# TaceoLabs/collaborative-circom

Hardware: AMD Instinct MI355X
Metric: Groth16 constraints/sec (BN254, 2^22 R1CS), one REP3 party's prove (higher is better)
Workload: dtype u32; 1 GPU; synthetic R1CS 2^22 constraints-domain BN254, REP3 co-groth16 (configs[2]); num_constraints=4194302, domain_size=4194304, nnz=12582906, msm=8 G1 + 2 G2 of ~2^22 points, ntt=12

## Files before the change

collaborative-circom_amd/csrc/capi_internal.hpp:

```cpp
#pragma once
#include "common.hpp"
#include "launchers.hpp"
#include "curve.hpp"
#include "subgroup.hpp"
#include "host_ec64.hpp"
#include "ntt_kernels.hpp"
#include "plonk_kernels.hpp"

#include <cmath>
#include <chrono>
#include <map>
#include <set>
#include <mutex>
#include <vector>

using namespace cg;

hipError_t hip_malloc_flush(void** p, size_t bytes);
template <class T> hipError_t hip_malloc_flush(T** p, size_t bytes) { return hip_malloc_flush((void**)p, bytes); }

namespace cgi {

struct Arena {
    char* base = nullptr; size_t cap = 0, used = 0;
    void* take(size_t bytes) { void* p = base + used; used += align_up(bytes); return p; }
};

enum { TW_BITREV = 1, TW_NATURAL = 2 };
struct TwKey { int curve; int log_m; uint32_t gen[8]; int kind = 0;
    bool operator<(const TwKey& o) const { if (curve != o.curve) return curve < o.curve; if (log_m != o.log_m) return log_m < o.log_m; if (kind != o.kind) return kind < o.kind; return memcmp(gen, o.gen, sizeof gen) < 0; } };
struct CosetKey { TwKey k; uint32_t scale[8]; bool operator<(const CosetKey& o) const { if (k < o.k) return true; if (o.k < k) return false; return memcmp(scale, o.scale, sizeof scale) < 0; } };
struct CosetTables { void* lo; void* hi; int log_lo; };

enum { TAG_MSM = 0, TAG_NTT, TAG_VEC, TAG_SPMV, TAG_SORT, TAG_ACC_G1, TAG_ACC_G2, TAG_REDUCE, TAG_COUNT };
struct EvPair { hipEvent_t a, b; int tag; };

struct MsmTicket {
    bool live = false;
    int curve = 0, group = 0, k = 0, c = 0, nwin = 0;
    uint32_t* h_flags = nullptr; bool optimistic = false;
    const cg_bases* bases = nullptr; size_t offset = 0, n = 0; std::vector<const void*> scalars;
    int nsums = 0;
    bool plain_fold = false;
    bool bit_fold = false;
    bool grid_fold = false; int log_l = 0, log_h = 0; uint32_t gc = 1, gr = 1;
    void* h_pinned = nullptr; size_t pinned_bytes = 0;
    hipEvent_t done = nullptr;
};

}
using namespace cgi;


struct cg_ctx {
    int device = 0;
    hipStream_t stream = nullptr;
    bool owns_stream = true;
    hipStream_t aux = nullptr;
    static constexpr int ACC_SLOTS_MAX = 8;
    hipEvent_t ev_acc[ACC_SLOTS_MAX] = {}, ev_red[ACC_SLOTS_MAX] = {};
    bool slot_busy[ACC_SLOTS_MAX] = {};
// ... 158 lines not shown
```

collaborative-circom_amd/csrc/capi_ntt.hip:

```cpp
#include "capi_internal.hpp"

namespace {
template <class Fr>
void host_pow_tables(const Fr& w, const Fr& first, int log_lo, size_t hi_n, std::vector<Fr>& lo, std::vector<Fr>& hi) {
    lo.resize((size_t)1 << log_lo); hi.resize(hi_n);
    Fr acc = first, step = Fr::one();
    for (size_t j = 0; j < lo.size(); j++) { lo[j] = acc; acc = acc * w; step = step * w; }
    Fr h = Fr::one();
    for (size_t j = 0; j < hi_n; j++) { hi[j] = h; h = h * step; }
}

struct SharedTwiddles { void* p; size_t bytes; int refs; uint64_t stamp; };
std::mutex g_tw_mu;
std::map<std::pair<int, TwKey>, SharedTwiddles> g_tw;
uint64_t g_tw_clock = 0;
void* shared_twiddles_acquire(int device, const TwKey& key) {
    std::lock_guard<std::mutex> l(g_tw_mu);
    auto it = g_tw.find({device, key});
    if (it == g_tw.end()) return nullptr;
    it->second.refs++; it->second.stamp = ++g_tw_clock;
    return it->second.p;
}
void* shared_twiddles_publish(int device, const TwKey& key, void* p, size_t bytes) {
    std::lock_guard<std::mutex> l(g_tw_mu);
// ... 49 lines not shown
    HIPCHK(hipStreamSynchronize(ctx->stream));
    HIPCHK(hipFree(d_lo)); HIPCHK(hipFree(d_hi));
    d_tw = shared_twiddles_publish(ctx->device, key, d_tw, bytes);
    ctx->twiddles[key] = d_tw;
    *out = d_tw;
    return 0;
}

template <class Fr>
int get_coset_tables(cg_ctx* ctx, int curve, int log_m, const Fr& g, const Fr& scale, CosetTables* out) {
    CosetKey key; key.k.curve = curve; key.k.log_m = log_m; memcpy(key.k.gen, g.v, sizeof key.k.gen); memcpy(key.scale, scale.v, sizeof key.scale);
    auto it = ctx->cosets.find(key);
    if (it != ctx->cosets.end()) { *out = it->second; return 0; }
    const size_t m = (size_t)1 << log_m;
    const int log_lo = std::min(11, log_m);
    const size_t hi_n = std::max<size_t>(1, m >> log_lo);
    std::vector<Fr> lo, hi;
    host_pow_tables(g, scale, log_lo, hi_n, lo, hi);
    CosetTables t; t.log_lo = log_lo;
    HIPCHK(hip_malloc_flush(&t.lo, lo.size() * sizeof(Fr)));
    HIPCHK(hip_malloc_flush(&t.hi, hi.size() * sizeof(Fr)));
    HIPCHK(hipMemcpy(t.lo, lo.data(), lo.size() * sizeof(Fr), hipMemcpyHostToDevice));
    HIPCHK(hipMemcpy(t.hi, hi.data(), hi.size() * sizeof(Fr), hipMemcpyHostToDevice));
    if (ctx->cosets.size() >= 64) {
        HIPCHK(hipStreamSynchronize(ctx->stream));
        for (auto& kv : ctx->cosets) { hipFree(kv.second.lo); hipFree(kv.second.hi); }
        ctx->cosets.clear();
    }
    ctx->cosets[key] = t;
    *out = t;
    return 0;
}

struct NttPass { int s0, k, t; };
std::vector<NttPass> ntt_plan(int log_m, int tile_log) {
    std::vector<NttPass> plan;
    const int k_last = std::min(log_m, tile_log);
    const int rest = log_m - k_last;
    int s0 = 0;
    if (rest > 0) {
        const int np = (rest + 6) / 7;
        for (int i = 0; i < np; i++) {
            int k = rest / np + (i < rest % np ? 1 : 0);
            plan.push_back({s0, k, tile_log - k});
            s0 += k;
        }
    }
    plan.push_back({s0, k_last, 0});
    return plan;
}

int ntt_lazy_tile() {
    static const int tile = [] { const char* e = tune_env("CG_NTT_TILE"); const int v = e ? atoi(e) : NTT_TILE_LOG_LAZY; return std::min(NTT_TILE_LOG, std::max(8, v)); }();
    return tile;
}

template <class Fr>
int ntt_run(cg_ctx* ctx, int curve, void* const* d_vecs, int k, size_t n, const Fr& gen, bool inverse, const Fr* coset, size_t arena_off) {
    const int log_m = log2_floor(n);
    if (((size_t)1 << log_m) != n) return fail(CG_ERR_ARG, "NTT length must be a power of two");
    if (k < 1 || k > NTT_MAX_VECS) return fail(CG_ERR_ARG, "k out of range");
    if (n == 1) return 0;
    if (!inverse && coset) return fail(CG_ERR_ARG, "coset_gen is only supported with inverse != 0");
    const Fr w = inverse ? fp_inverse(gen) : gen;
    const void* twl = nullptr;
    int rc = get_twiddles_lazy<Fr>(ctx, curve, log_m, w, false, &twl);
    if (rc) return rc;
    NttVecs data{}, tmp{};
    for (int j = 0; j < k; j++) { data.p[j] = d_vecs[j]; tmp.p[j] = ctx->ntt_arena.base + arena_off + (size_t)j * lazy29_bytes(n); }
    hipStream_t st = ctx->stream;
    bool first = true;
    for (const NttPass& p : ntt_plan(log_m, ntt_lazy_tile())) { rc = launch_ntt_ct_pass<Fr>(st, first, first ? data : tmp, tmp, k, n, log_m, p.s0, p.k, p.t, twl); if (rc) return rc; first = false; }
    const Fr scale32 = inverse ? mont32<Fr>() * inv_pow2<Fr>(log_m) : mont32<Fr>();
    CosetTables t;
    const Fr* d_scale = nullptr; const Fr* c_lo = nullptr; const Fr* c_hi = nullptr; int log_lo = 0;
    if (coset) { rc = get_coset_tables<Fr>(ctx, curve, log_m, *coset, scale32, &t); if (rc) return rc; c_lo = (const Fr*)t.lo; c_hi = (const Fr*)t.hi; log_lo = t.log_lo; }
    else { rc = get_coset_tables<Fr>(ctx, curve, 0, Fr::one(), scale32, &t); if (rc) return rc; d_scale = (const Fr*)t.lo; }
    return launch_bitrev_finish_lazy<Fr>(st, data, tmp, k, n, log_m, d_scale, c_lo, c_hi, log_lo);
}

template <class Fr>
int ntt_coset_pair_run(cg_ctx* ctx, int curve, void* const* d_vecs, int k, size_t n, const Fr& gen, const Fr& coset, size_t arena_off) {
    const int log_m = log2_floor(n);
    if (((size_t)1 << log_m) != n) return fail(CG_ERR_ARG, "NTT length must be a power of two");
    if (k < 1 || k > NTT_MAX_VECS) return fail(CG_ERR_ARG, "k out of range");
    if (n == 1) return 0;
    const void* tw_inv = nullptr; const void* tw_fwd = nullptr;
    int rc = get_twiddles_lazy<Fr>(ctx, curve, log_m, fp_inverse(gen), false, &tw_inv); if (rc) return rc;
    rc = get_twiddles_lazy<Fr>(ctx, curve, log_m, gen, true, &tw_fwd); if (rc) return rc;
    const Fr c32 = mont32<Fr>();
    CosetTables ct;
    rc = get_coset_tables<Fr>(ctx, curve, log_m, coset, c32 * inv_pow2<Fr>(log_m), &ct); if (rc) return rc;
    NttVecs data{}, tmp{};
    for (int j = 0; j < k; j++) { data.p[j] = d_vecs[j]; tmp.p[j] = ctx->ntt_arena.base + arena_off + (size_t)j * lazy29_bytes(n); }
    hipStream_t st = ctx->stream;
    const std::vector<NttPass> plan = ntt_plan(log_m, ntt_lazy_tile());
    bool first = true;
    for (const NttPass& p : plan) { rc = launch_ntt_ct_pass<Fr>(st, first, first ? data : tmp, tmp, k, n, log_m, p.s0, p.k, p.t, tw_inv); if (rc) return rc; first = false; }
    for (size_t i = plan.size(); i-- > 0;) {
        const NttPass& p = plan[i];
        rc = launch_ntt_dit_pass<Fr>(st, i + 1 == plan.size(), i == 0, data, tmp, k, n, log_m, p.s0, p.k, p.t, tw_fwd, (const Fr*)ct.lo, (const Fr*)ct.hi, ct.log_lo, c32);
        if (rc) return rc;
    }
    return 0;
}

}

extern "C" {
int32_t cg_ntt_dev(cg_ctx* ctx, int32_t curve, void* const* d_vecs, int32_t k, size_t n, const void* h_group_gen, int32_t inverse, const void* h_coset_gen) {
    if (!ctx || !d_vecs || !h_group_gen) return fail(CG_ERR_ARG, "null argument");
    HIPCHK(hipSetDevice(ctx->device));
    return with_fr(curve, [&](auto tag) -> int {
        typedef decltype(tag) Fr;
        Fr gen, cos; copy_in(gen, h_group_gen);
        if (h_coset_gen) copy_in(cos, h_coset_gen);
        if (n > 1) { int rc = ensure_ntt_arena(ctx, (size_t)k * lazy29_bytes(n)); if (rc) return rc; }
        StatScope ss(ctx, TAG_NTT);
        return ntt_run<Fr>(ctx, curve, d_vecs, k, n, gen, inverse != 0, h_coset_gen ? &cos : nullptr, 0);
    });
}
int32_t cg_ntt_coset_pair_dev(cg_ctx* ctx, int32_t curve, void* const* d_vecs, int32_t k, size_t n, const void* h_group_gen, const void* h_coset_gen) {
    if (!ctx || !d_vecs || !h_group_gen || !h_coset_gen) return fail(CG_ERR_ARG, "null argument");
    HIPCHK(hipSetDevice(ctx->device));
    return with_fr(curve, [&](auto tag) -> int {
        typedef decltype(tag) Fr;
        Fr gen, cos; copy_in(gen, h_group_gen); copy_in(cos, h_coset_gen);
        if (n > 1) { int rc = ensure_ntt_arena(ctx, (size_t)k * lazy29_bytes(n)); if (rc) return rc; }
        StatScope ss(ctx, TAG_NTT);
        return ntt_coset_pair_run<Fr>(ctx, curve, d_vecs, k, n, gen, cos, 0);
    });
}
int32_t cg_ntt(cg_ctx* ctx, int32_t curve, void* const* h_vecs, int32_t k, size_t n, const void* h_group_gen, int32_t inverse, const void* h_coset_gen) {
    if (!ctx || !h_vecs) return fail(CG_ERR_ARG, "null argument");
// ... 28 lines not shown
```

collaborative-circom_amd/csrc/fr_impl.hpp:

```cpp
#pragma once
#include "launchers.hpp"
#include "ntt_kernels.hpp"
#include "vec_kernels.hpp"
#include "plonk_kernels.hpp"
#include "r1cs_kernels.hpp"
#include "plonk_setup_kernels.hpp"
#include "msm_sort_kernels.hpp"

namespace cg {

template <class Fr> int launch_vec_binary(hipStream_t st, int op, Fr* out, const Fr* a, const Fr* b, size_t n) {
    if (!n) return 0;
    if (op == 0) hipLaunchKernelGGL((k_vec_binary<Fr, 0>), dim3(grid_for(n)), dim3(256), 0, st, out, a, b, n);
    else if (op == 1) hipLaunchKernelGGL((k_vec_binary<Fr, 1>), dim3(grid_for(n)), dim3(256), 0, st, out, a, b, n);
    else hipLaunchKernelGGL((k_vec_binary<Fr, 2>), dim3(grid_for(n)), dim3(256), 0, st, out, a, b, n);
    HIPCHK(hipGetLastError());
    return 0;
}
template <class Fr> int launch_rep3_mul_local(hipStream_t st, Fr* out, const Fr* aa, const Fr* ab, const Fr* ba, const Fr* bb, const Fr* mask, size_t n) {
    if (!n) return 0;
    hipLaunchKernelGGL((k_rep3_mul_local<Fr>), dim3(grid_for(n)), dim3(256), 0, st, out, aa, ab, ba, bb, mask, n);
    HIPCHK(hipGetLastError());
    return 0;
}
// ... 129 lines not shown
    for (int i = 0; i < 5; i++) if (n > n_constraints) HIPCHK(hipMemsetAsync((Fr*)o.q[i] + n_constraints, 0, (n - n_constraints) * sizeof(Fr), st));
    if (n_rows + n_public) hipLaunchKernelGGL((k_plonk_gate_emit<Fr>), dim3(grid_for(n_rows + n_public)), dim3(256), 0, st, A, B, C, n_rows, n_wires, n_public, counts, offsets, o);
    HIPCHK(hipGetLastError());
    return 0;
}
template <class Fr> int launch_plonk_sigma_labels(hipStream_t st, const uint32_t* prev, const Fr* wpow, int log_n, const Fr& k1, const Fr& k2, Fr* sigma) {
    hipLaunchKernelGGL((k_plonk_sigma_labels<Fr>), dim3(grid_for((size_t)3 << log_n)), dim3(256), 0, st, prev, wpow, log_n, k1, k2, sigma);
    HIPCHK(hipGetLastError());
    return 0;
}
template <class Fr> int launch_build_twiddles_lazy(hipStream_t st, void* tw, size_t m, int log_m, const Fr* lo, const Fr* hi, int log_lo, const Fr& c32) {
    if (m > 1) hipLaunchKernelGGL((k_build_twiddles_lazy<Fr>), dim3(grid_for(m / 2)), dim3(256), 0, st, tw, m / 2, log_m, lo, hi, log_lo, c32);
    HIPCHK(hipGetLastError());
    return 0;
}
template <class Fr> int launch_ntt_ct_pass(hipStream_t st, bool first, NttVecs src, NttVecs dst, int nvec, size_t n, int log_m, int s0, int k, int t, const void* tw) {
    static PerDeviceOnce attr_set;
    if (attr_set.pending()) {
        HIPCHK(hipFuncSetAttribute((const void*)k_ntt_ct_pass<Fr, true>, hipFuncAttributeMaxDynamicSharedMemorySize, 36 << NTT_TILE_LOG));
        HIPCHK(hipFuncSetAttribute((const void*)k_ntt_ct_pass<Fr, false>, hipFuncAttributeMaxDynamicSharedMemorySize, 36 << NTT_TILE_LOG));
        attr_set.mark();
    }
    const int E = 1 << (k + t);
    if (first) hipLaunchKernelGGL((k_ntt_ct_pass<Fr, true>), dim3((unsigned)(n / E), nvec), dim3(NTT_THREADS), (size_t)E * 36, st, src, dst, log_m, s0, k, t, tw);
    else hipLaunchKernelGGL((k_ntt_ct_pass<Fr, false>), dim3((unsigned)(n / E), nvec), dim3(NTT_THREADS), (size_t)E * 36, st, src, dst, log_m, s0, k, t, tw);
    HIPCHK(hipGetLastError());
    return 0;
}
template <class Fr> int launch_build_twiddles_lazy_natural(hipStream_t st, void* tw, size_t m, const Fr* lo, const Fr* hi, int log_lo, const Fr& c32) {
    if (m > 1) hipLaunchKernelGGL((k_build_twiddles_lazy_natural<Fr>), dim3(grid_for(m / 2)), dim3(256), 0, st, tw, m / 2, lo, hi, log_lo, c32);
    HIPCHK(hipGetLastError());
    return 0;
}
template <class Fr> int launch_ntt_dit_pass(hipStream_t st, bool first, bool last, NttVecs out, NttVecs tmp, int nvec, size_t n, int log_m, int s0, int k, int t, const void* tw,
                                            const Fr* c_lo, const Fr* c_hi, int log_lo, const Fr& c32) {
    static PerDeviceOnce attr_set;
    if (attr_set.pending()) {
        HIPCHK(hipFuncSetAttribute((const void*)k_ntt_dit_pass<Fr, true, true>, hipFuncAttributeMaxDynamicSharedMemorySize, 36 << NTT_TILE_LOG));
        HIPCHK(hipFuncSetAttribute((const void*)k_ntt_dit_pass<Fr, true, false>, hipFuncAttributeMaxDynamicSharedMemorySize, 36 << NTT_TILE_LOG));
        HIPCHK(hipFuncSetAttribute((const void*)k_ntt_dit_pass<Fr, false, true>, hipFuncAttributeMaxDynamicSharedMemorySize, 36 << NTT_TILE_LOG));
        HIPCHK(hipFuncSetAttribute((const void*)k_ntt_dit_pass<Fr, false, false>, hipFuncAttributeMaxDynamicSharedMemorySize, 36 << NTT_TILE_LOG));
        attr_set.mark();
    }
    const int E = 1 << (k + t);
    const dim3 grid((unsigned)(n / E), nvec); const size_t lds = (size_t)E * 36;
    if (first && last) hipLaunchKernelGGL((k_ntt_dit_pass<Fr, true, true>), grid, dim3(NTT_THREADS), lds, st, out, tmp, log_m, s0, k, t, tw, c_lo, c_hi, log_lo, c32);
    else if (first) hipLaunchKernelGGL((k_ntt_dit_pass<Fr, true, false>), grid, dim3(NTT_THREADS), lds, st, out, tmp, log_m, s0, k, t, tw, c_lo, c_hi, log_lo, c32);
    else if (last) hipLaunchKernelGGL((k_ntt_dit_pass<Fr, false, true>), grid, dim3(NTT_THREADS), lds, st, out, tmp, log_m, s0, k, t, tw, c_lo, c_hi, log_lo, c32);
    else hipLaunchKernelGGL((k_ntt_dit_pass<Fr, false, false>), grid, dim3(NTT_THREADS), lds, st, out, tmp, log_m, s0, k, t, tw, c_lo, c_hi, log_lo, c32);
    HIPCHK(hipGetLastError());
    return 0;
}
template <class Fr> int launch_bitrev_finish_lazy(hipStream_t st, NttVecs dst, NttVecs src, int nvec, size_t n, int log_m, const Fr* scale, const Fr* c_lo, const Fr* c_hi, int log_lo) {
    if (log_m >= 2 * BITREV_B_LAZY)
        hipLaunchKernelGGL((k_bitrev_finish_lazy<Fr>), dim3((unsigned)(n >> (2 * BITREV_B_LAZY)), nvec), dim3(256), 0, st, dst, src, log_m, scale, c_lo, c_hi, log_lo);
    else
        hipLaunchKernelGGL((k_bitrev_finish_lazy_small<Fr>), dim3(grid_for(n), nvec), dim3(256), 0, st, dst, src, log_m, scale, c_lo, c_hi, log_lo);
    HIPCHK(hipGetLastError());
    return 0;
}

inline bool msm_sort_use_partition(size_t n, int c, int nwin, int shared) {
    const size_t nbuckets = (size_t)(shared ? 1 : nwin) << (c - 1);
    const size_t nregions = (nbuckets + ((size_t)1 << PART_REGION_LOG) - 1) >> PART_REGION_LOG;
    return (size_t)nwin * n >= ((size_t)1 << 21) && nregions >= 8 && nregions <= PART_MAX_REGIONS;
}
template <class Fr> int msm_sort_launch(hipStream_t st, const Fr* d_scalars, size_t n, int c, int nwin, int shared, char* scratch, MsmSortPtrs* out, hipEvent_t* evs) {
    const size_t nbuckets = (size_t)(shared ? 1 : nwin) << (c - 1);
    size_t off = 0;
    auto take = [&](size_t bytes) { void* p = scratch + off; off += align_up(bytes); return p; };
    int32_t* digits = (int32_t*)take((size_t)nwin * n * 4);
    uint32_t* sorted = (uint32_t*)take((size_t)nwin * n * 4);
    uint32_t* counts = (uint32_t*)take(nbuckets * 4);
    uint32_t* cursors = (uint32_t*)take(nbuckets * 4);
    uint32_t* offsets = (uint32_t*)take(nbuckets * 4);
    const size_t ntiles = (nbuckets + SCAN_TILE - 1) / SCAN_TILE;
    uint32_t* tile_sums = (uint32_t*)take(ntiles * 4);
    if (evs) HIPCHK(hipEventRecord(evs[0], st));
    const bool no_small = !global_option(CG_GOPT_SORT_SMALL);
    static PerDeviceOnce attr_small; static std::atomic<bool> small_unavailable{false};
    if (shared && !no_small && !small_unavailable.load(std::memory_order_relaxed) && attr_small.pending()) {
        if (hipFuncSetAttribute((const void*)k_msm_sort_small<Fr>, hipFuncAttributeMaxDynamicSharedMemorySize, (int)((2 * SORT_SMALL_MAX_BUCKETS + 1024) * 4)) == hipSuccess) attr_small.mark();
// ... 78 lines not shown
}

#define CG_INSTANTIATE_FR(Fr)                                                                                              \
    namespace cg {                                                                                                         \
    template decltype(launch_vec_binary<Fr>) launch_vec_binary<Fr>;                                                        \
    template decltype(launch_rep3_mul_local<Fr>) launch_rep3_mul_local<Fr>;                                                \
    template decltype(launch_distribute_powers<Fr>) launch_distribute_powers<Fr>;                                          \
    template decltype(launch_vec_count_noncanonical<Fr>) launch_vec_count_noncanonical<Fr>;                                \
    template decltype(launch_vec_fill<Fr>) launch_vec_fill<Fr>;                                                            \
    template decltype(launch_vec_gather_idx<Fr>) launch_vec_gather_idx<Fr>;                                                \
    template decltype(launch_vec_affine<Fr>) launch_vec_affine<Fr>;                                                        \
    template decltype(launch_vec_gather_strided<Fr>) launch_vec_gather_strided<Fr>;                                        \
    template decltype(launch_vec_lincomb<Fr>) launch_vec_lincomb<Fr>;                                                      \
    template decltype(launch_shamir_share<Fr>) launch_shamir_share<Fr>;                                                    \
    template decltype(launch_plonk_r2_factors<Fr>) launch_plonk_r2_factors<Fr>;                                            \
    template decltype(launch_prefix_scan<Fr>) launch_prefix_scan<Fr>;                                                      \
    template decltype(launch_vec_inverse<Fr>) launch_vec_inverse<Fr>;                                                      \
    template decltype(launch_plonk_additions<Fr>) launch_plonk_additions<Fr>;                                              \
    template decltype(launch_plonk_r3_blind<Fr>) launch_plonk_r3_blind<Fr>;                                                \
    template decltype(launch_plonk_r3_perm<Fr>) launch_plonk_r3_perm<Fr>;                                                  \
    template decltype(launch_plonk_r3_gate<Fr>) launch_plonk_r3_gate<Fr>;                                                  \
    template decltype(launch_plonk_mul4_tail<Fr>) launch_plonk_mul4_tail<Fr>;                                              \
    template decltype(launch_plonk_r3_t<Fr>) launch_plonk_r3_t<Fr>;                                                        \
    template decltype(launch_plonk_r3_divide<Fr>) launch_plonk_r3_divide<Fr>;                                              \
    template decltype(launch_spmv_csr<Fr>) launch_spmv_csr<Fr>;                                                            \
    template decltype(launch_r1cs_check<Fr>) launch_r1cs_check<Fr>;                                                        \
    template decltype(launch_qap_columns<Fr>) launch_qap_columns<Fr>;                                                      \
    template decltype(launch_plonk_gate_count<Fr>) launch_plonk_gate_count<Fr>;                                            \
    template decltype(launch_plonk_gate_emit<Fr>) launch_plonk_gate_emit<Fr>;                                              \
    template decltype(launch_plonk_sigma_labels<Fr>) launch_plonk_sigma_labels<Fr>;                                        \
    template decltype(launch_build_twiddles_lazy<Fr>) launch_build_twiddles_lazy<Fr>;                                      \
    template decltype(launch_ntt_ct_pass<Fr>) launch_ntt_ct_pass<Fr>;                                                      \
    template decltype(launch_build_twiddles_lazy_natural<Fr>) launch_build_twiddles_lazy_natural<Fr>;                      \
    template decltype(launch_ntt_dit_pass<Fr>) launch_ntt_dit_pass<Fr>;                                                    \
    template decltype(launch_bitrev_finish_lazy<Fr>) launch_bitrev_finish_lazy<Fr>;                                        \
    template decltype(msm_sort_launch<Fr>) msm_sort_launch<Fr>;                                                            \
    template decltype(msm_sort_direct_launch<Fr>) msm_sort_direct_launch<Fr>;                                              \
    }
```

collaborative-circom_amd/csrc/launchers.hpp:

```cpp
#pragma once
#include "common.hpp"

namespace cg {

template <class F> struct Affine;
template <class F> struct XYZZ;
template <class F> struct FastSubgroup;
struct NttVecs;
template <class F> struct PlonkR2Args;
template <class F> struct PlonkBlindArgs;
template <class F> struct PlonkPermArgs;
template <class F> struct PlonkGateArgs;
template <class F> struct PlonkMul4Args;
template <class F> struct PlonkTArgs;
template <class F> struct PlonkDivArgs;

constexpr int SCAN_TILE = 2048;
constexpr int PART_TILE = 16384;
constexpr int PART_REGION_LOG = 9;
constexpr int PART_MAX_REGIONS = 4096;
struct MsmSortPtrs { const uint32_t* sorted; const uint32_t* offsets; const uint32_t* counts; uint32_t cap; const uint32_t* overflow; };
inline size_t msm_sort_scratch_bytes(size_t n, int c, int nwin) {
    const size_t nbuckets = (size_t)nwin << (c - 1);
    const size_t entries = (size_t)nwin * n;
// ... 32 lines not shown
template <class Fr> int launch_vec_fill(hipStream_t st, Fr* v, size_t n, const Fr& value);
template <class Fr> int launch_vec_gather_strided(hipStream_t st, Fr* out, const Fr* in, size_t n, size_t offset, size_t stride);
template <class Fr> int launch_prefix_scan(hipStream_t st, int op, Fr* out, const Fr* in, size_t n, Fr* scratch);
template <class Fr> int launch_vec_inverse(hipStream_t st, Fr* out, const Fr* in, size_t n);
template <class Fr> int launch_spmv_csr(hipStream_t st, const uint32_t* row_ptr, const uint32_t* col, const Fr* coeff, size_t n_rows, const Fr* pub,
                                        uint32_t n_inputs, int party, const Fr* wit_a, const Fr* wit_b, Fr* out_a, Fr* out_b);
struct R1csMat { const uint32_t* row_ptr; const uint32_t* col; const void* coeff; };
constexpr uint32_t QAP_LONG_COLUMN = 64;
template <class Fr> int launch_r1cs_check(hipStream_t st, const R1csMat& A, const R1csMat& B, const R1csMat& C, size_t n_rows, size_t nnz_total, int form, const Fr* w,
                                          unsigned long long* result);
template <class Fr> int launch_qap_columns(hipStream_t st, const uint32_t* col_ptr, const uint32_t* row, const Fr* coeff, size_t n_cols, const Fr* L, Fr* out, uint32_t long_min);
struct PlonkGateOut {
    uint32_t* map[3];
    void* q[5];
    uint32_t* add_ids;
    void* add_f;
};
template <class Fr> int launch_plonk_gate_count(hipStream_t st, const R1csMat& A, const R1csMat& B, const R1csMat& C, size_t n_rows, uint32_t* counts, uint32_t* offsets, uint32_t* tile_sums);
template <class Fr> int launch_plonk_gate_emit(hipStream_t st, const R1csMat& A, const R1csMat& B, const R1csMat& C, size_t n_rows, uint32_t n_wires, uint32_t n_public,
                                               const uint32_t* counts, const uint32_t* offsets, size_t n_constraints, size_t n, const PlonkGateOut& o);
template <class Fr> int launch_plonk_sigma_labels(hipStream_t st, const uint32_t* prev, const Fr* wpow, int log_n, const Fr& k1, const Fr& k2, Fr* sigma);
template <class Fr> int launch_plonk_additions(hipStream_t st, const uint32_t* order, size_t n, const uint32_t* ids, const Fr* coeffs, const Fr* pub, uint32_t n_inputs, int pc,
                                               Fr* ext_a, Fr* ext_b, size_t n_priv);
template <class Fr> int launch_plonk_r2_factors(hipStream_t st, const PlonkR2Args<Fr>& g, size_t n);
template <class Fr> int launch_plonk_r3_blind(hipStream_t st, const PlonkBlindArgs<Fr>& g, size_t n);
template <class Fr> int launch_plonk_r3_perm(hipStream_t st, const PlonkPermArgs<Fr>& g, size_t n);
template <class Fr> int launch_plonk_r3_gate(hipStream_t st, const PlonkGateArgs<Fr>& g, size_t n);
template <class Fr> int launch_plonk_mul4_tail(hipStream_t st, const PlonkMul4Args<Fr>& g, size_t n);
template <class Fr> int launch_plonk_r3_t(hipStream_t st, const PlonkTArgs<Fr>& g, size_t n);
template <class Fr> int launch_plonk_r3_divide(hipStream_t st, const PlonkDivArgs<Fr>& g, size_t n);
template <class Fr> int launch_build_twiddles_lazy(hipStream_t st, void* tw, size_t m, int log_m, const Fr* lo, const Fr* hi, int log_lo, const Fr& c32);
template <class Fr> int launch_build_twiddles_lazy_natural(hipStream_t st, void* tw, size_t m, const Fr* lo, const Fr* hi, int log_lo, const Fr& c32);
template <class Fr> int launch_ntt_ct_pass(hipStream_t st, bool first, NttVecs src, NttVecs dst, int nvec, size_t n, int log_m, int s0, int k, int t, const void* tw);
template <class Fr> int launch_ntt_dit_pass(hipStream_t st, bool first, bool last, NttVecs out, NttVecs tmp, int nvec, size_t n, int log_m, int s0, int k, int t, const void* tw,
                                            const Fr* c_lo, const Fr* c_hi, int log_lo, const Fr& c32);
template <class Fr> int launch_bitrev_finish_lazy(hipStream_t st, NttVecs dst, NttVecs src, int nvec, size_t n, int log_m, const Fr* scale, const Fr* c_lo, const Fr* c_hi, int log_lo);

int chacha12_fr_rand_launch(hipStream_t st, const uint32_t* key8, const uint32_t* mod8, int modulus_bits, uint64_t word_pos, uint64_t n_pairs, uint64_t n,
                            void* d_cand, uint32_t* d_tiles, unsigned long long* d_result, void* d_out);

}
```

collaborative-circom_amd/csrc/lazy29.hpp:

```cpp
#pragma once
#include "field.hpp"

namespace cg {

template <class F> struct XYZZ;

template <class F>
struct L29 {
    typedef typename F::Params P;
    static constexpr int NL = F::N == 8 ? 9 : 14;
    static constexpr int W = F::N == 8 ? 29 : 28;
    static constexpr int SH = NL * W - 32 * F::N;
    static constexpr int TOPBIT = W * (NL - 1);
    static_assert(F::N == 8 || F::N == 12, "");
    static constexpr uint32_t MASK = (1u << W) - 1;
    int32_t l[NL];

    static constexpr int32_t pl(int k) {
        const int bit = W * k, w = bit >> 5, sh = bit & 31;
        const uint64_t two = (w < F::N ? (uint64_t)P::P[w] : 0) | (w + 1 < F::N ? (uint64_t)P::P[w + 1] << 32 : 0);
        return (int32_t)((uint32_t)(two >> sh) & MASK);
    }
    template <int SHIFT>
    __device__ __forceinline__ static L29 unpack(const F& a) {
// ... 191 lines not shown
        }
        return upper_half(T);
    }
    __device__ __forceinline__ static XYZZ<F> dbl_affine(const F& x, const F& y) { return xyzz_dbl_affine(x, y); }
    __device__ __forceinline__ static L29 one() { const L29 o = unpack<SH>(F::one()); return mul(o, o); }
    __device__ __forceinline__ static L29 one_small() {
        L29 o = unpack_small(F::one());
        L29 pp; _Pragma("unroll") for (int k = 0; k < NL; k++) pp.l[k] = pl(k);
        const L29 t = (o + pp).norm();
        if (o.l[NL - 1] < 0) o = t;
        return o;
    }
    __device__ __forceinline__ static F to_fp(const L29& x) {
        L29 c; _Pragma("unroll") for (int k = 0; k < NL; k++) c.l[k] = 0;
        c.l[(32 * F::N) / W] = 1 << ((32 * F::N) % W);
        return pack_reduced(mul(x, c));
    }
    __device__ __forceinline__ static F pack_reduced(L29 y) {
        L29 pp; _Pragma("unroll") for (int k = 0; k < NL; k++) pp.l[k] = pl(k);
        L29 t = (y + pp).norm();
        if (y.l[NL - 1] < 0) y = t;
        t = (y - pp).norm();
        if (t.l[NL - 1] >= 0) y = t;
        F r;
        _Pragma("unroll") for (int w = 0; w < F::N; w++) {
            const int k = (32 * w) / W, sh = 32 * w - W * k;
            uint64_t v = (uint64_t)(uint32_t)y.l[k] >> sh;
            if (k + 1 < NL) v |= (uint64_t)(uint32_t)y.l[k + 1] << (W - sh);
            if (k + 2 < NL && 2 * W - sh < 32) v |= (uint64_t)(uint32_t)y.l[k + 2] << (2 * W - sh);
            r.v[w] = (uint32_t)v;
        }
        return r;
    }
};

}
```

collaborative-circom_amd/csrc/ntt_kernels.hpp:

```cpp
#pragma once
#include "field.hpp"
#include "lazy29.hpp"
#include "vec_kernels.hpp"

namespace cg {

constexpr int NTT_MAX_VECS = 8;
struct NttVecs { void* p[NTT_MAX_VECS]; };

constexpr int NTT_TILE_LOG = 11;
constexpr int NTT_THREADS = 256;
constexpr int NTT_TILE_LOG_LAZY = 10;
constexpr int BITREV_B_LAZY = 5;

struct Lazy29Planes { uint4* p0; uint4* p1; uint32_t* p2; };
__host__ __device__ inline size_t lazy29_bytes(size_t n) { return ((n * 36 + 255) / 256) * 256; }
__device__ __forceinline__ Lazy29Planes lazy29_planes(void* base, size_t n) {
    char* b = reinterpret_cast<char*>(base);
    return {reinterpret_cast<uint4*>(b), reinterpret_cast<uint4*>(b + n * 16), reinterpret_cast<uint32_t*>(b + n * 32)};
}
template <class L> __device__ __forceinline__ L lazy29_load(const uint4* p0, const uint4* p1, const uint32_t* p2, size_t i) {
    const uint4 x = p0[i], y = p1[i]; L r;
    r.l[0] = (int32_t)x.x; r.l[1] = (int32_t)x.y; r.l[2] = (int32_t)x.z; r.l[3] = (int32_t)x.w;
    r.l[4] = (int32_t)y.x; r.l[5] = (int32_t)y.y; r.l[6] = (int32_t)y.z; r.l[7] = (int32_t)y.w; r.l[8] = (int32_t)p2[i];
// ... 14 lines not shown
        const F w = ld_fp(lo + (e & (((size_t)1 << log_lo) - 1))) * ld_fp(hi + (e >> log_lo)) * c32;
        lazy29_store<L>(tw.p0, tw.p1, tw.p2, i, L::template unpack<0>(w));
    }
}

template <class F, bool FIRST>
__global__ void __launch_bounds__(NTT_THREADS) k_ntt_ct_pass(NttVecs src_vecs, NttVecs dst_vecs, int log_m, int s0, int k, int t, const void* tw_base) {
    static_assert(F::N == 8, "NTT is specialised for 256-bit scalar fields");
    typedef L29<F> L;
    extern __shared__ uint4 lds[];
    const int E = 1 << (k + t);
    uint4* pl0 = lds;
    uint4* pl1 = lds + E;
    uint32_t* pl2 = reinterpret_cast<uint32_t*>(lds + 2 * E);
    const size_t m = (size_t)1 << log_m;
    const Lazy29Planes tw = lazy29_planes(const_cast<void*>(tw_base), m / 2);
    const Lazy29Planes dst = lazy29_planes(dst_vecs.p[blockIdx.y], m);
    const int lo_bits = log_m - s0 - k;
    const size_t tiles_per_hi = (size_t)1 << (lo_bits - t);
    const size_t hi = blockIdx.x / tiles_per_hi;
    const size_t lo0 = (blockIdx.x % tiles_per_hi) << t;
    const size_t base = (hi << (log_m - s0)) + lo0;
    const int tmask = (1 << t) - 1;

    for (int idx = threadIdx.x; idx < E; idx += NTT_THREADS) {
        const size_t g = base + ((size_t)(idx >> t) << lo_bits) + (idx & tmask);
        L v;
        if constexpr (FIRST) v = L::template unpack<0>(ld_fp(reinterpret_cast<const F*>(src_vecs.p[blockIdx.y]) + g));
        else v = lazy29_load<L>(dst.p0, dst.p1, dst.p2, g);
        lazy29_store<L>(pl0, pl1, pl2, idx, v);
    }
    __syncthreads();
    int q = 0;
    for (; q + 1 < k; q += 2) {
        const int pb = k - 1 - q;
        for (int u = threadIdx.x; u < E / 4; u += NTT_THREADS) {
            const int lo_local = u & tmask;
            const int mu = u >> t;
            const int mid0 = ((mu >> (pb - 1)) << (pb + 1)) | (mu & ((1 << (pb - 1)) - 1));
            const int i00 = (mid0 << t) | lo_local, d0 = 1 << (pb + t), d1 = 1 << (pb - 1 + t);
            const size_t blk = (hi << q) | (size_t)(mid0 >> (k - q));
            L a0 = lazy29_load<L>(pl0, pl1, pl2, i00), a1 = lazy29_load<L>(pl0, pl1, pl2, i00 + d1);
            const L a2 = lazy29_load<L>(pl0, pl1, pl2, i00 + d0), a3 = lazy29_load<L>(pl0, pl1, pl2, i00 + d0 + d1);
            const L w = lazy29_load<L>(tw.p0, tw.p1, tw.p2, blk);
            L v2, v3; L::mul2_cols(a2, w, a3, w, v2, v3);
            const L b0 = a0 + v2, b2 = a0 - v2;
            const L b1 = (a1 + v3).norm(), b3 = (a1 - v3).norm();
            const L w0 = lazy29_load<L>(tw.p0, tw.p1, tw.p2, 2 * blk), w1 = lazy29_load<L>(tw.p0, tw.p1, tw.p2, 2 * blk + 1);
            L y1, y3; L::mul2_cols(b1, w0, b3, w1, y1, y3);
            lazy29_store<L>(pl0, pl1, pl2, i00, (b0 + y1).norm());
            lazy29_store<L>(pl0, pl1, pl2, i00 + d1, (b0 - y1).norm());
            lazy29_store<L>(pl0, pl1, pl2, i00 + d0, (b2 + y3).norm());
            lazy29_store<L>(pl0, pl1, pl2, i00 + d0 + d1, (b2 - y3).norm());
        }
        __syncthreads();
    }
    for (; q < k; q++) {
        const int pb = k - 1 - q;
        for (int u = threadIdx.x; u < E / 2; u += NTT_THREADS) {
            const int lo_local = u & tmask;
            const int mu = u >> t;
            const int mid0 = ((mu >> pb) << (pb + 1)) | (mu & ((1 << pb) - 1));
            const int i0 = (mid0 << t) | lo_local;
            const int i1 = i0 + (1 << (pb + t));
            const size_t blk = (hi << q) | (size_t)(mid0 >> (k - q));
            const L a = lazy29_load<L>(pl0, pl1, pl2, i0), b = lazy29_load<L>(pl0, pl1, pl2, i1);
            const L w = lazy29_load<L>(tw.p0, tw.p1, tw.p2, blk);
            const L v = L::mul_cols(b, w);
            lazy29_store<L>(pl0, pl1, pl2, i0, (a + v).norm());
            lazy29_store<L>(pl0, pl1, pl2, i1, (a - v).norm());
        }
        __syncthreads();
    }
    for (int idx = threadIdx.x; idx < E; idx += NTT_THREADS) {
        const size_t g = base + ((size_t)(idx >> t) << lo_bits) + (idx & tmask);
        lazy29_store<L>(dst.p0, dst.p1, dst.p2, g, lazy29_load<L>(pl0, pl1, pl2, idx));
    }
}

template <class F>
__global__ void __launch_bounds__(256) k_build_twiddles_lazy_natural(void* tw_base, size_t half, const F* __restrict__ lo, const F* __restrict__ hi, int log_lo, F c32) {
    typedef L29<F> L;
    const Lazy29Planes tw = lazy29_planes(tw_base, half);
    for (size_t e = (size_t)blockIdx.x * blockDim.x + threadIdx.x; e < half; e += (size_t)gridDim.x * blockDim.x) {
        const F w = ld_fp(lo + (e & (((size_t)1 << log_lo) - 1))) * ld_fp(hi + (e >> log_lo)) * c32;
        lazy29_store<L>(tw.p0, tw.p1, tw.p2, e, L::template unpack<0>(w));
    }
}
template <class F, bool FIRST, bool LAST>
__global__ void __launch_bounds__(NTT_THREADS) k_ntt_dit_pass(NttVecs out_vecs, NttVecs tmp_vecs, int log_m, int s0, int k, int t, const void* tw_base,
                                                             const F* __restrict__ cos_lo, const F* __restrict__ cos_hi, int log_lo, F c32) {
    static_assert(F::N == 8, "NTT is specialised for 256-bit scalar fields");
    typedef L29<F> L;
    extern __shared__ uint4 lds[];
    const int E = 1 << (k + t);
    uint4* pl0 = lds;
    uint4* pl1 = lds + E;
    uint32_t* pl2 = reinterpret_cast<uint32_t*>(lds + 2 * E);
    const size_t m = (size_t)1 << log_m;
    const Lazy29Planes tw = lazy29_planes(const_cast<void*>(tw_base), m / 2);
    const Lazy29Planes buf = lazy29_planes(tmp_vecs.p[blockIdx.y], m);
    const int lo_bits = log_m - s0 - k;
    const size_t tiles_per_hi = (size_t)1 << (lo_bits - t);
    const size_t hi = blockIdx.x / tiles_per_hi;
    const size_t lo0 = (blockIdx.x % tiles_per_hi) << t;
    const size_t base = (hi << (log_m - s0)) + lo0;
    const int tmask = (1 << t) - 1;

    for (int idx = threadIdx.x; idx < E; idx += NTT_THREADS) {
        const size_t g = base + ((size_t)(idx >> t) << lo_bits) + (idx & tmask);
        L v = lazy29_load<L>(buf.p0, buf.p1, buf.p2, g);
        if constexpr (FIRST) {
            const size_t i = (size_t)(__brevll((unsigned long long)g) >> (64 - log_m));
            const F c = ld_fp(cos_lo + (i & (((size_t)1 << log_lo) - 1))) * ld_fp(cos_hi + (i >> log_lo));
            v = L::mul_cols(v, L::template unpack<0>(c));
        }
        lazy29_store<L>(pl0, pl1, pl2, idx, v);
    }
    __syncthreads();
    int q = 0;
    for (; q + 1 < k; q += 2) {
        const int s = lo_bits + q;
        for (int u = threadIdx.x; u < E / 4; u += NTT_THREADS) {
            const int lo_local = u & tmask;
            const int mu = u >> t;
            const int mid0 = ((mu >> q) << (q + 2)) | (mu & ((1 << q) - 1));
            const int i00 = (mid0 << t) | lo_local, d = 1 << (q + t);
            const size_t j = ((size_t)(mid0 & ((1 << q) - 1)) << lo_bits) + lo0 + lo_local;
            const size_t e0 = j << (log_m - 1 - s), e1 = j << (log_m - 2 - s);
            const L a00 = lazy29_load<L>(pl0, pl1, pl2, i00), a01 = lazy29_load<L>(pl0, pl1, pl2, i00 + d);
            const L a10 = lazy29_load<L>(pl0, pl1, pl2, i00 + 2 * d), a11 = lazy29_load<L>(pl0, pl1, pl2, i00 + 3 * d);
            const L w0 = lazy29_load<L>(tw.p0, tw.p1, tw.p2, e0);
            L v1, v3; L::mul2_cols(a01, w0, a11, w0, v1, v3);
            const L b00 = a00 + v1, b01 = a00 - v1;
            const L b10 = (a10 + v3).norm(), b11 = (a10 - v3).norm();
            const L w1a = lazy29_load<L>(tw.p0, tw.p1, tw.p2, e1), w1b = lazy29_load<L>(tw.p0, tw.p1, tw.p2, e1 + (m >> 2));
            L y2, y3; L::mul2_cols(b10, w1a, b11, w1b, y2, y3);
            lazy29_store<L>(pl0, pl1, pl2, i00, (b00 + y2).norm());
            lazy29_store<L>(pl0, pl1, pl2, i00 + 2 * d, (b00 - y2).norm());
            lazy29_store<L>(pl0, pl1, pl2, i00 + d, (b01 + y3).norm());
            lazy29_store<L>(pl0, pl1, pl2, i00 + 3 * d, (b01 - y3).norm());
        }
        __syncthreads();
    }
    for (; q < k; q++) {
        const int s = lo_bits + q;
        for (int u = threadIdx.x; u < E / 2; u += NTT_THREADS) {
            const int lo_local = u & tmask;
            const int mu = u >> t;
            const int mid0 = ((mu >> q) << (q + 1)) | (mu & ((1 << q) - 1));
            const int i0 = (mid0 << t) | lo_local, i1 = i0 + (1 << (q + t));
            const size_t j = ((size_t)(mid0 & ((1 << q) - 1)) << lo_bits) + lo0 + lo_local;
            const L a = lazy29_load<L>(pl0, pl1, pl2, i0), b = lazy29_load<L>(pl0, pl1, pl2, i1);
            const L v = L::mul_cols(b, lazy29_load<L>(tw.p0, tw.p1, tw.p2, j << (log_m - 1 - s)));
            lazy29_store<L>(pl0, pl1, pl2, i0, (a + v).norm());
            lazy29_store<L>(pl0, pl1, pl2, i1, (a - v).norm());
        }
        __syncthreads();
    }
    for (int idx = threadIdx.x; idx < E; idx += NTT_THREADS) {
        const size_t g = base + ((size_t)(idx >> t) << lo_bits) + (idx & tmask);
        const L v = lazy29_load<L>(pl0, pl1, pl2, idx);
        if constexpr (LAST) st_fp(reinterpret_cast<F*>(out_vecs.p[blockIdx.y]) + g, L::pack_reduced(L::mul_cols(v, L::template unpack<0>(c32))));
        else lazy29_store<L>(buf.p0, buf.p1, buf.p2, g, v);
    }
}

template <class F>
__global__ void __launch_bounds__(256) k_bitrev_finish_lazy(NttVecs dst, NttVecs src, int log_m, const F* __restrict__ scale,
                                                            const F* __restrict__ cos_lo, const F* __restrict__ cos_hi, int log_lo) {
    typedef L29<F> L;
    constexpr int B = BITREV_B_LAZY, S = 1 << B;
    __shared__ uint4 tile0[S * (S + 1)];
    __shared__ uint4 tile1[S * (S + 1)];
    __shared__ uint32_t tile2[S * (S + 1)];
    const size_t m = (size_t)1 << log_m;
    const Lazy29Planes in = lazy29_planes(src.p[blockIdx.y], m);
    F* out = reinterpret_cast<F*>(dst.p[blockIdx.y]);
    const int mid_bits = log_m - 2 * B;
    const size_t mid = blockIdx.x;
    const size_t rmid = mid_bits > 0 ? (__brevll((unsigned long long)mid) >> (64 - mid_bits)) : 0;
    for (int e = threadIdx.x; e < S * S; e += 256) {
        const int h = e >> B, l = e & (S - 1);
        const size_t i = ((size_t)h << (log_m - B)) | (mid << B) | (size_t)l;
        tile0[h * (S + 1) + l] = in.p0[i]; tile1[h * (S + 1) + l] = in.p1[i]; tile2[h * (S + 1) + l] = in.p2[i];
    }
    __syncthreads();
    for (int e = threadIdx.x; e < S * S; e += 256) {
        const int rl = e >> B, rh = e & (S - 1);
        const int l = __brev((unsigned)rl) >> (32 - B), h = __brev((unsigned)rh) >> (32 - B);
        const size_t o = ((size_t)rl << (log_m - B)) | (rmid << B) | (size_t)rh;
        const L v = lazy29_load<L>(tile0, tile1, tile2, (size_t)(h * (S + 1) + l));
        const F c = cos_lo ? ld_fp(cos_lo + (o & (((size_t)1 << log_lo) - 1))) * ld_fp(cos_hi + (o >> log_lo)) : ld_fp(scale);
        st_fp(out + o, L::pack_reduced(L::mul_cols(v, L::template unpack<0>(c))));
    }
}
// ... 17 lines not shown
```

Before: 61.31 million constraints/s.

## Precompute lazy coset table, specialize trivial-twiddle first stages, drop final Montgomery multiply

```diff
diff --git a/collaborative-circom_amd/csrc/capi_internal.hpp b/collaborative-circom_amd/csrc/capi_internal.hpp
--- a/collaborative-circom_amd/csrc/capi_internal.hpp
+++ b/collaborative-circom_amd/csrc/capi_internal.hpp
@@ -26,7 +26,7 @@
     void* take(size_t bytes) { void* p = base + used; used += align_up(bytes); return p; }
 };
 
-enum { TW_BITREV = 1, TW_NATURAL = 2 };
+enum { TW_BITREV = 1, TW_NATURAL = 2, TW_COSET = 3 };
 struct TwKey { int curve; int log_m; uint32_t gen[8]; int kind = 0;
     bool operator<(const TwKey& o) const { if (curve != o.curve) return curve < o.curve; if (log_m != o.log_m) return log_m < o.log_m; if (kind != o.kind) return kind < o.kind; return memcmp(gen, o.gen, sizeof gen) < 0; } };
 struct CosetKey { TwKey k; uint32_t scale[8]; bool operator<(const CosetKey& o) const { if (k < o.k) return true; if (o.k < k) return false; return memcmp(scale, o.scale, sizeof scale) < 0; } };
diff --git a/collaborative-circom_amd/csrc/capi_ntt.hip b/collaborative-circom_amd/csrc/capi_ntt.hip
--- a/collaborative-circom_amd/csrc/capi_ntt.hip
+++ b/collaborative-circom_amd/csrc/capi_ntt.hip
@@ -105,6 +105,27 @@
     return 0;
 }
 
+template <class Fr>
+int get_coset_lazy(cg_ctx* ctx, int curve, int log_m, const Fr& g, const void** out) {
+    TwKey key; key.curve = curve; key.log_m = log_m; key.kind = TW_COSET; memcpy(key.gen, g.v, sizeof key.gen);
+    auto it = ctx->twiddles.find(key);
+    if (it != ctx->twiddles.end()) { *out = it->second; return 0; }
+    if (void* shared = shared_twiddles_acquire(ctx->device, key)) { ctx->twiddles[key] = shared; *out = shared; return 0; }
+    CosetTables ct;
+    int rc = get_coset_tables<Fr>(ctx, curve, log_m, g, mont32<Fr>() * inv_pow2<Fr>(log_m), &ct); if (rc) return rc;
+    const size_t m = (size_t)1 << log_m;
+    const size_t bytes = lazy29_bytes(m);
+    void* d_cos = nullptr;
+    HIPCHK(hip_malloc_flush(&d_cos, bytes));
+    rc = launch_build_coset_lazy<Fr>(ctx->stream, d_cos, m, log_m, (const Fr*)ct.lo, (const Fr*)ct.hi, ct.log_lo);
+    if (rc) { hipFree(d_cos); return rc; }
+    HIPCHK(hipStreamSynchronize(ctx->stream));
+    d_cos = shared_twiddles_publish(ctx->device, key, d_cos, bytes);
+    ctx->twiddles[key] = d_cos;
+    *out = d_cos;
+    return 0;
+}
+
 struct NttPass { int s0, k, t; };
 std::vector<NttPass> ntt_plan(int log_m, int tile_log) {
     std::vector<NttPass> plan;
@@ -161,9 +182,8 @@
     const void* tw_inv = nullptr; const void* tw_fwd = nullptr;
     int rc = get_twiddles_lazy<Fr>(ctx, curve, log_m, fp_inverse(gen), false, &tw_inv); if (rc) return rc;
     rc = get_twiddles_lazy<Fr>(ctx, curve, log_m, gen, true, &tw_fwd); if (rc) return rc;
-    const Fr c32 = mont32<Fr>();
-    CosetTables ct;
-    rc = get_coset_tables<Fr>(ctx, curve, log_m, coset, c32 * inv_pow2<Fr>(log_m), &ct); if (rc) return rc;
+    const void* cos = nullptr;
+    rc = get_coset_lazy<Fr>(ctx, curve, log_m, coset, &cos); if (rc) return rc;
     NttVecs data{}, tmp{};
     for (int j = 0; j < k; j++) { data.p[j] = d_vecs[j]; tmp.p[j] = ctx->ntt_arena.base + arena_off + (size_t)j * lazy29_bytes(n); }
     hipStream_t st = ctx->stream;
@@ -172,7 +192,7 @@
     for (const NttPass& p : plan) { rc = launch_ntt_ct_pass<Fr>(st, first, first ? data : tmp, tmp, k, n, log_m, p.s0, p.k, p.t, tw_inv); if (rc) return rc; first = false; }
     for (size_t i = plan.size(); i-- > 0;) {
         const NttPass& p = plan[i];
-        rc = launch_ntt_dit_pass<Fr>(st, i + 1 == plan.size(), i == 0, data, tmp, k, n, log_m, p.s0, p.k, p.t, tw_fwd, (const Fr*)ct.lo, (const Fr*)ct.hi, ct.log_lo, c32);
+        rc = launch_ntt_dit_pass<Fr>(st, i + 1 == plan.size(), i == 0, data, tmp, k, n, log_m, p.s0, p.k, p.t, tw_fwd, cos);
         if (rc) return rc;
     }
     return 0;
diff --git a/collaborative-circom_amd/csrc/fr_impl.hpp b/collaborative-circom_amd/csrc/fr_impl.hpp
--- a/collaborative-circom_amd/csrc/fr_impl.hpp
+++ b/collaborative-circom_amd/csrc/fr_impl.hpp
@@ -185,8 +185,12 @@
     HIPCHK(hipGetLastError());
     return 0;
 }
-template <class Fr> int launch_ntt_dit_pass(hipStream_t st, bool first, bool last, NttVecs out, NttVecs tmp, int nvec, size_t n, int log_m, int s0, int k, int t, const void* tw,
-                                            const Fr* c_lo, const Fr* c_hi, int log_lo, const Fr& c32) {
+template <class Fr> int launch_build_coset_lazy(hipStream_t st, void* cos, size_t m, int log_m, const Fr* lo, const Fr* hi, int log_lo) {
+    hipLaunchKernelGGL((k_build_coset_lazy<Fr>), dim3(grid_for(m)), dim3(256), 0, st, cos, m, log_m, lo, hi, log_lo);
+    HIPCHK(hipGetLastError());
+    return 0;
+}
+template <class Fr> int launch_ntt_dit_pass(hipStream_t st, bool first, bool last, NttVecs out, NttVecs tmp, int nvec, size_t n, int log_m, int s0, int k, int t, const void* tw, const void* cos) {
     static PerDeviceOnce attr_set;
     if (attr_set.pending()) {
         HIPCHK(hipFuncSetAttribute((const void*)k_ntt_dit_pass<Fr, true, true>, hipFuncAttributeMaxDynamicSharedMemorySize, 36 << NTT_TILE_LOG));
@@ -197,10 +201,10 @@
     }
     const int E = 1 << (k + t);
     const dim3 grid((unsigned)(n / E), nvec); const size_t lds = (size_t)E * 36;
-    if (first && last) hipLaunchKernelGGL((k_ntt_dit_pass<Fr, true, true>), grid, dim3(NTT_THREADS), lds, st, out, tmp, log_m, s0, k, t, tw, c_lo, c_hi, log_lo, c32);
-    else if (first) hipLaunchKernelGGL((k_ntt_dit_pass<Fr, true, false>), grid, dim3(NTT_THREADS), lds, st, out, tmp, log_m, s0, k, t, tw, c_lo, c_hi, log_lo, c32);
-    else if (last) hipLaunchKernelGGL((k_ntt_dit_pass<Fr, false, true>), grid, dim3(NTT_THREADS), lds, st, out, tmp, log_m, s0, k, t, tw, c_lo, c_hi, log_lo, c32);
-    else hipLaunchKernelGGL((k_ntt_dit_pass<Fr, false, false>), grid, dim3(NTT_THREADS), lds, st, out, tmp, log_m, s0, k, t, tw, c_lo, c_hi, log_lo, c32);
+    if (first && last) hipLaunchKernelGGL((k_ntt_dit_pass<Fr, true, true>), grid, dim3(NTT_THREADS), lds, st, out, tmp, log_m, s0, k, t, tw, cos);
+    else if (first) hipLaunchKernelGGL((k_ntt_dit_pass<Fr, true, false>), grid, dim3(NTT_THREADS), lds, st, out, tmp, log_m, s0, k, t, tw, cos);
+    else if (last) hipLaunchKernelGGL((k_ntt_dit_pass<Fr, false, true>), grid, dim3(NTT_THREADS), lds, st, out, tmp, log_m, s0, k, t, tw, cos);
+    else hipLaunchKernelGGL((k_ntt_dit_pass<Fr, false, false>), grid, dim3(NTT_THREADS), lds, st, out, tmp, log_m, s0, k, t, tw, cos);
     HIPCHK(hipGetLastError());
     return 0;
 }
@@ -345,6 +349,7 @@
     template decltype(launch_build_twiddles_lazy<Fr>) launch_build_twiddles_lazy<Fr>;                                      \
     template decltype(launch_ntt_ct_pass<Fr>) launch_ntt_ct_pass<Fr>;                                                      \
     template decltype(launch_build_twiddles_lazy_natural<Fr>) launch_build_twiddles_lazy_natural<Fr>;                      \
+    template decltype(launch_build_coset_lazy<Fr>) launch_build_coset_lazy<Fr>;                                            \
     template decltype(launch_ntt_dit_pass<Fr>) launch_ntt_dit_pass<Fr>;                                                    \
     template decltype(launch_bitrev_finish_lazy<Fr>) launch_bitrev_finish_lazy<Fr>;                                        \
     template decltype(msm_sort_launch<Fr>) msm_sort_launch<Fr>;                                                            \
diff --git a/collaborative-circom_amd/csrc/launchers.hpp b/collaborative-circom_amd/csrc/launchers.hpp
--- a/collaborative-circom_amd/csrc/launchers.hpp
+++ b/collaborative-circom_amd/csrc/launchers.hpp
@@ -88,8 +88,8 @@
 template <class Fr> int launch_build_twiddles_lazy(hipStream_t st, void* tw, size_t m, int log_m, const Fr* lo, const Fr* hi, int log_lo, const Fr& c32);
 template <class Fr> int launch_build_twiddles_lazy_natural(hipStream_t st, void* tw, size_t m, const Fr* lo, const Fr* hi, int log_lo, const Fr& c32);
 template <class Fr> int launch_ntt_ct_pass(hipStream_t st, bool first, NttVecs src, NttVecs dst, int nvec, size_t n, int log_m, int s0, int k, int t, const void* tw);
-template <class Fr> int launch_ntt_dit_pass(hipStream_t st, bool first, bool last, NttVecs out, NttVecs tmp, int nvec, size_t n, int log_m, int s0, int k, int t, const void* tw,
-                                            const Fr* c_lo, const Fr* c_hi, int log_lo, const Fr& c32);
+template <class Fr> int launch_build_coset_lazy(hipStream_t st, void* cos, size_t m, int log_m, const Fr* lo, const Fr* hi, int log_lo);
+template <class Fr> int launch_ntt_dit_pass(hipStream_t st, bool first, bool last, NttVecs out, NttVecs tmp, int nvec, size_t n, int log_m, int s0, int k, int t, const void* tw, const void* cos);
 template <class Fr> int launch_bitrev_finish_lazy(hipStream_t st, NttVecs dst, NttVecs src, int nvec, size_t n, int log_m, const Fr* scale, const Fr* c_lo, const Fr* c_hi, int log_lo);
 
 int chacha12_fr_rand_launch(hipStream_t st, const uint32_t* key8, const uint32_t* mod8, int modulus_bits, uint64_t word_pos, uint64_t n_pairs, uint64_t n,
diff --git a/collaborative-circom_amd/csrc/lazy29.hpp b/collaborative-circom_amd/csrc/lazy29.hpp
--- a/collaborative-circom_amd/csrc/lazy29.hpp
+++ b/collaborative-circom_amd/csrc/lazy29.hpp
@@ -247,6 +247,24 @@
         }
         return r;
     }
+    static constexpr int RS_OFF = 128, RS_MAX = 127;
+    static constexpr int32_t rs_top() {
+        int64_t c = 0;
+        for (int j = 0; j < NL - 1; j++) c = ((int64_t)RS_OFF * pl(j) + c) >> W;
+        return (int32_t)((int64_t)RS_OFF * pl(NL - 1) + c);
+    }
+    __device__ __forceinline__ static F reduce_pack(const L29& x) {
+        static_assert(F::N == 8, "the offset is sized for the 256-bit fields");
+        const uint32_t top = (uint32_t)(x.l[NL - 1] + rs_top());
+        const int32_t kk = (int32_t)(((uint64_t)top * quot_c()) >> QS) - RS_OFF;
+        L29 r; int64_t c = 0;
+        _Pragma("unroll") for (int j = 0; j < NL; j++) {
+            const int64_t t = (int64_t)x.l[j] - (int64_t)kk * pl(j) + c;
+            r.l[j] = j < NL - 1 ? (int32_t)((uint32_t)t & MASK) : (int32_t)t;
+            c = t >> W;
+        }
+        return pack_reduced(r);
+    }
 };
 
 }
diff --git a/collaborative-circom_amd/csrc/ntt_kernels.hpp b/collaborative-circom_amd/csrc/ntt_kernels.hpp
--- a/collaborative-circom_amd/csrc/ntt_kernels.hpp
+++ b/collaborative-circom_amd/csrc/ntt_kernels.hpp
@@ -70,6 +70,37 @@
     }
     __syncthreads();
     int q = 0;
+    if constexpr (FIRST) {
+        if (k >= 2) {
+            const int pb = k - 1;
+            for (int u = threadIdx.x; u < E / 4; u += NTT_THREADS) {
+                const int lo_local = u & tmask;
+                const int mu = u >> t;
+                const int mid0 = ((mu >> (pb - 1)) << (pb + 1)) | (mu & ((1 << (pb - 1)) - 1));
+                const int i00 = (mid0 << t) | lo_local, d0 = 1 << (pb + t), d1 = 1 << (pb - 1 + t);
+                const L a0 = lazy29_load<L>(pl0, pl1, pl2, i00), a1 = lazy29_load<L>(pl0, pl1, pl2, i00 + d1);
+                const L a2 = lazy29_load<L>(pl0, pl1, pl2, i00 + d0), a3 = lazy29_load<L>(pl0, pl1, pl2, i00 + d0 + d1);
+                const L b0 = a0 + a2, b2 = a0 - a2, b1 = a1 + a3;
+                const L b3 = (a1 - a3).norm();
+                const L y3 = L::mul_cols(b3, lazy29_load<L>(tw.p0, tw.p1, tw.p2, 1));
+                lazy29_store<L>(pl0, pl1, pl2, i00, (b0 + b1).norm());
+                lazy29_store<L>(pl0, pl1, pl2, i00 + d1, (b0 - b1).norm());
+                lazy29_store<L>(pl0, pl1, pl2, i00 + d0, (b2 + y3).norm());
+                lazy29_store<L>(pl0, pl1, pl2, i00 + d0 + d1, (b2 - y3).norm());
+            }
+            __syncthreads();
+            q = 2;
+        } else {
+            for (int u = threadIdx.x; u < E / 2; u += NTT_THREADS) {
+                const int i0 = u & tmask, i1 = i0 + (1 << t);
+                const L a = lazy29_load<L>(pl0, pl1, pl2, i0), b = lazy29_load<L>(pl0, pl1, pl2, i1);
+                lazy29_store<L>(pl0, pl1, pl2, i0, (a + b).norm());
+                lazy29_store<L>(pl0, pl1, pl2, i1, (a - b).norm());
+            }
+            __syncthreads();
+            q = 1;
+        }
+    }
     for (; q + 1 < k; q += 2) {
         const int pb = k - 1 - q;
         for (int u = threadIdx.x; u < E / 4; u += NTT_THREADS) {
@@ -125,9 +156,18 @@
         lazy29_store<L>(tw.p0, tw.p1, tw.p2, e, L::template unpack<0>(w));
     }
 }
+template <class F>
+__global__ void __launch_bounds__(256) k_build_coset_lazy(void* cos_base, size_t m, int log_m, const F* __restrict__ lo, const F* __restrict__ hi, int log_lo) {
+    typedef L29<F> L;
+    const Lazy29Planes cos = lazy29_planes(cos_base, m);
+    for (size_t g = (size_t)blockIdx.x * blockDim.x + threadIdx.x; g < m; g += (size_t)gridDim.x * blockDim.x) {
+        const size_t i = (size_t)(__brevll((unsigned long long)g) >> (64 - log_m));
+        const F c = ld_fp(lo + (i & (((size_t)1 << log_lo) - 1))) * ld_fp(hi + (i >> log_lo));
+        lazy29_store<L>(cos.p0, cos.p1, cos.p2, g, L::template unpack<0>(c));
+    }
+}
 template <class F, bool FIRST, bool LAST>
-__global__ void __launch_bounds__(NTT_THREADS) k_ntt_dit_pass(NttVecs out_vecs, NttVecs tmp_vecs, int log_m, int s0, int k, int t, const void* tw_base,
-                                                             const F* __restrict__ cos_lo, const F* __restrict__ cos_hi, int log_lo, F c32) {
+__global__ void __launch_bounds__(NTT_THREADS) k_ntt_dit_pass(NttVecs out_vecs, NttVecs tmp_vecs, int log_m, int s0, int k, int t, const void* tw_base, const void* cos_base) {
     static_assert(F::N == 8, "NTT is specialised for 256-bit scalar fields");
     typedef L29<F> L;
     extern __shared__ uint4 lds[];
@@ -138,6 +178,7 @@
     const size_t m = (size_t)1 << log_m;
     const Lazy29Planes tw = lazy29_planes(const_cast<void*>(tw_base), m / 2);
     const Lazy29Planes buf = lazy29_planes(tmp_vecs.p[blockIdx.y], m);
+    const Lazy29Planes cos = lazy29_planes(const_cast<void*>(cos_base), m);
     const int lo_bits = log_m - s0 - k;
     const size_t tiles_per_hi = (size_t)1 << (lo_bits - t);
     const size_t hi = blockIdx.x / tiles_per_hi;
@@ -148,15 +189,37 @@
     for (int idx = threadIdx.x; idx < E; idx += NTT_THREADS) {
         const size_t g = base + ((size_t)(idx >> t) << lo_bits) + (idx & tmask);
         L v = lazy29_load<L>(buf.p0, buf.p1, buf.p2, g);
-        if constexpr (FIRST) {
-            const size_t i = (size_t)(__brevll((unsigned long long)g) >> (64 - log_m));
-            const F c = ld_fp(cos_lo + (i & (((size_t)1 << log_lo) - 1))) * ld_fp(cos_hi + (i >> log_lo));
-            v = L::mul_cols(v, L::template unpack<0>(c));
-        }
+        if constexpr (FIRST) v = L::mul_cols(v, lazy29_load<L>(cos.p0, cos.p1, cos.p2, g));
         lazy29_store<L>(pl0, pl1, pl2, idx, v);
     }
     __syncthreads();
     int q = 0;
+    if constexpr (FIRST) {
+        if (k >= 2) {
+            for (int u = threadIdx.x; u < E / 4; u += NTT_THREADS) {
+                const int i00 = u << 2;
+                const L a00 = lazy29_load<L>(pl0, pl1, pl2, i00), a01 = lazy29_load<L>(pl0, pl1, pl2, i00 + 1);
+                const L a10 = lazy29_load<L>(pl0, pl1, pl2, i00 + 2), a11 = lazy29_load<L>(pl0, pl1, pl2, i00 + 3);
+                const L b00 = a00 + a01, b01 = a00 - a01, b10 = a10 + a11;
+                const L b11 = (a10 - a11).norm();
+                const L y3 = L::mul_cols(b11, lazy29_load<L>(tw.p0, tw.p1, tw.p2, m >> 2));
+                lazy29_store<L>(pl0, pl1, pl2, i00, (b00 + b10).norm());
+                lazy29_store<L>(pl0, pl1, pl2, i00 + 2, (b00 - b10).norm());
+                lazy29_store<L>(pl0, pl1, pl2, i00 + 1, (b01 + y3).norm());
+                lazy29_store<L>(pl0, pl1, pl2, i00 + 3, (b01 - y3).norm());
+            }
+            __syncthreads();
+            q = 2;
+        } else {
+            for (int u = threadIdx.x; u < E / 2; u += NTT_THREADS) {
+                const L a = lazy29_load<L>(pl0, pl1, pl2, 2 * u), b = lazy29_load<L>(pl0, pl1, pl2, 2 * u + 1);
+                lazy29_store<L>(pl0, pl1, pl2, 2 * u, (a + b).norm());
+                lazy29_store<L>(pl0, pl1, pl2, 2 * u + 1, (a - b).norm());
+            }
+            __syncthreads();
+            q = 1;
+        }
+    }
     for (; q + 1 < k; q += 2) {
         const int s = lo_bits + q;
         for (int u = threadIdx.x; u < E / 4; u += NTT_THREADS) {
@@ -199,7 +262,7 @@
     for (int idx = threadIdx.x; idx < E; idx += NTT_THREADS) {
         const size_t g = base + ((size_t)(idx >> t) << lo_bits) + (idx & tmask);
         const L v = lazy29_load<L>(pl0, pl1, pl2, idx);
-        if constexpr (LAST) st_fp(reinterpret_cast<F*>(out_vecs.p[blockIdx.y]) + g, L::pack_reduced(L::mul_cols(v, L::template unpack<0>(c32))));
+        if constexpr (LAST) st_fp(reinterpret_cast<F*>(out_vecs.p[blockIdx.y]) + g, L::reduce_pack(v));
         else lazy29_store<L>(buf.p0, buf.p1, buf.p2, g, v);
     }
 }
```

After: 61.71 million constraints/s, median of 6. No clear change (+0.7%).
